# instadeepai/FrameDiPT

Hardware: AMD Instinct MI355X
Metric: residue*diffusion-steps/sec (higher is better)
Workload: dtype fp16

## Files before the change

framedipt_amd/_lib.py:

```python
from __future__ import annotations

import ctypes as C
import os

_HERE = os.path.dirname(os.path.abspath(__file__))
LIB_PATH = os.environ.get("FDIPT_LIB") or os.path.join(_HERE, "lib", "libfdipt_hip.so")

PREC_F32, PREC_BF16, PREC_F16 = 0, 1, 2
KF_ET3, KF_GENERIC_PAIR, KF_GENERIC_ATTN, KF_UNFUSED_NODE, KF_UNFOLDED, KF_NO_SPLIT, KF_NO_MERGE, KF_ROWS32, KF_PASS_Z = 1, 2, 4, 8, 16, 32, 64, 128, 256
_ERR = {-1: "FDIPT_EINVAL (bad argument)", -2: "FDIPT_ELAUNCH (HIP launch error)",
        -3: "FDIPT_ESIZE (workspace too small or N beyond the compiled tiling)"}


class FdiptError(RuntimeError):
    pass


class Dims(C.Structure):
    _fields_ = [(n, C.c_int32) for n in (
        "c_s", "c_z", "c_hidden", "c_skip", "no_heads", "no_qk_points", "no_v_points", "tfmr_heads", "tfmr_layers",
        "num_blocks", "index_embed", "num_bins", "use_aatype", "precision", "kernel_flags")] + [
        (n, C.c_float) for n in ("min_bin", "max_bin", "coordinate_scaling", "r3_min_b", "r3_max_b")]


_P = C.c_void_p


class ForwardArgs(C.Structure):
    _fields_ = [("B", C.c_int32), ("N", C.c_int32), ("n_rel", C.c_int32), ("rel_off", C.c_int32)] + [
        (n, _P) for n in ("rigids_t", "res_mask", "fixed_mask", "sc_ca_t", "seq_idx", "idx_emb", "aatype", "gt_psi", "t",
                          "t_emb", "t_emb_eps", "so3_sigma", "bb_tables", "psi", "rot_score", "trans_score", "rigids",
                          "atom37", "atom14", "trace_node", "trace_edge", "trace_inner")] + [
# ... 110 lines not shown
```

framedipt_amd/csrc/ipa_proj2.hip:

```cpp
#include <type_traits>

#include "common.hpp"
#include "kernels.hpp"

#define P2_K 256
#define P2_KS (P2_K / 16)
#define P2_WBLK (4 * P2_KS * 1024)
#define P2_XROW (P2_K * 2)
#define P2_LDS (2 * P2_WBLK)

typedef fd_h p2_hx2 __attribute__((ext_vector_type(2)));
typedef float p2_f32x2 __attribute__((ext_vector_type(2)));
typedef unsigned p2_u32x2 __attribute__((ext_vector_type(2)));
typedef unsigned p2_u32x4 __attribute__((ext_vector_type(4)));
__device__ __forceinline__ int p2_perm16(int pos) { return 4 * (pos >> 3) + (pos & 3) + 8 * ((pos & 7) >> 2); }
__device__ __forceinline__ void p2_dma16(const void* gsrc, unsigned lds_dst) {
  const unsigned m0v = __builtin_amdgcn_readfirstlane(lds_dst);
  asm volatile("s_mov_b32 m0, %0\n\ts_nop 0\n\tglobal_load_lds_dwordx4 %1, off" : : "s"(m0v), "v"(gsrc) : "memory", "m0");
}
typedef const __attribute__((address_space(3))) u16x8* p2_lds_u16x8;
typedef const __attribute__((address_space(3))) f32x4* p2_lds_f32x4;
typedef const __attribute__((address_space(3))) float* p2_lds_f32;
__device__ __forceinline__ hx8 p2_frag(unsigned off) { return __builtin_bit_cast(hx8, *(p2_lds_u16x8)(unsigned long)off); }

#define P2S_HALF 32768
#define P2S_STAGE (2 * P2S_HALF)
#define P2S_BIAS_OFF (2 * P2S_STAGE)
template <bool QK, bool SPLIT>
__device__ __forceinline__ void ipa_proj2_body(const ProjArgs& a, int n_cblk, int walker, int n_walkers, char* smem) {
  const unsigned lds0 = (unsigned)(unsigned long)(__attribute__((address_space(3))) char*)smem;
  const int tid = threadIdx.x, lane = tid & 63, wave = tid >> 6, li = lane & 31, hi = lane >> 5;
  constexpr int RB = SPLIT ? 256 : 128;
  constexpr int TM = SPLIT ? 1 : 2;
  constexpr int NTH = SPLIT ? 512 : FD_THREADS;
  const int wr = SPLIT ? wave : wave >> 1;
  int wc = SPLIT ? 0 : (wave & 1);
  const bool mrg = a.merged != 0;
  const int M = a.B * a.N, HC = a.H * a.C, NOUT = (mrg ? HC : 3 * HC) + a.PT, ntl = a.Np >> 5;
  const int m0 = blockIdx.x * RB;
  const char* wimg = (const char*)a.W_img;
  const char* wimg_lo = (const char*)a.W_img_lo;
  const int nq = HC / 128, per_head = (2 * a.C) / 128, n_class = mrg ? (QK ? nq : n_cblk - nq) : (QK ? 2 * nq : n_cblk - 2 * nq);
  auto cblk_of = [&](int k) {
    if (mrg) return QK ? k : nq + k;
    if (QK) return k < nq ? k : nq + ((k - nq) / (per_head / 2)) * per_head + (k - nq) % (per_head / 2);
    const int nv = nq;
    return k < nv ? nq + (k / (per_head / 2)) * per_head + per_head / 2 + k % (per_head / 2) : 3 * nq + (k - nv);
  };
  int kb = walker;
  auto request = [&](int c, int buf) {
// ... 60 lines not shown
    }
    __syncthreads();
  } else {
    char* xs = smem + P2_WBLK;
#pragma unroll
    for (int it = 0; it < 32; ++it) {
      const int idx = tid + it * FD_THREADS, r = idx >> 6, c4 = idx & 63;
      const int gr = m0 + r < M ? m0 + r : M - 1;
      const f32x4 x = *(const f32x4*)(a.A + (long)gr * a.lda + 4 * c4);
      const p2_u32x2 h = {fd_cvt_pk(x[0], x[1]), fd_cvt_pk(x[2], x[3])};
      *(p2_u32x2*)(xs + r * P2_XROW + (((c4 >> 1) ^ (r & 15)) << 4) + 8 * (c4 & 1)) = h;
    }
    __syncthreads();
#pragma unroll
    for (int i = 0; i < 2; ++i)
#pragma unroll
      for (int s = 0; s < P2_KS; ++s) {
        const int r = (wr * 2 + i) * 32 + li;
        Af[i][s] = p2_frag(lds0 + P2_WBLK + r * P2_XROW + (((2 * s + hi) ^ (r & 15)) << 4));
      }
    __builtin_amdgcn_s_waitcnt(0xC07F);
  }
  FD_STAMP(1);
  int qk_row[TM];
  int v_row[TM][4];
  int p_row[TM][4];
#pragma unroll
  for (int i = 0; i < TM; ++i) {
    const int m = m0 + (wr * TM + i) * 32 + li;
    const int b = m < M ? m / a.N : 0, r = m - b * a.N;
    qk_row[i] = m < M ? ((b * a.H * ntl + (r >> 5)) * (a.C >> 4) * 64 + (r & 31)) * 8 : -1;
#pragma unroll
    for (int g = 0; g < 4; ++g) {
      const int mg = m0 + (wr * TM + i) * 32 + 8 * g + 4 * hi;
      const int bb = mg < M ? mg / a.N : 0, key = mg - bb * a.N, pp = (key & ~15) + p2_perm16(key & 15);
      v_row[i][g] = mg + 3 < M ? (bb * a.H * (a.C >> 5) * (2 * ntl) + (pp >> 4)) * 512 + ((pp >> 3) & 1) * 256 + (pp & 7) : -1;
      p_row[i][g] = mg + 3 < M ? mg * a.PT : -1;
    }
  }
  auto epi_unit = [&](const f32x16 (&acc)[TM][2], const auto& BQ, const int (&cpart)[2], int kind, int i, int j, int g) {
    if constexpr (QK) {
      if ((g & 1) || qk_row[i] < 0) return;
      const f32x4 b0 = BQ.q(j, g), b1 = BQ.q(j, g + 1);
      const float sc = kind == 0 ? a.qscale : 1.f;
      const p2_u32x4 o = {fd_cvt_pk((acc[i][j][4 * g] + b0[0]) * sc, (acc[i][j][4 * g + 1] + b0[1]) * sc),
                          fd_cvt_pk((acc[i][j][4 * g + 2] + b0[2]) * sc, (acc[i][j][4 * g + 3] + b0[3]) * sc),
// ... 93 lines not shown
          acc[0][j] = fd_mfma32(l, Af[0][s], acc[0][j]);
          acc[0][j] = fd_mfma32(h, Al[0][s], acc[0][j]);
          acc[0][j] = fd_mfma32(h, Af[0][s], acc[0][j]);
        } else {
          acc[0][j] = fd_mfma32(Af[0][s], l, acc[0][j]);
          acc[0][j] = fd_mfma32(Al[0][s], h, acc[0][j]);
          acc[0][j] = fd_mfma32(Af[0][s], h, acc[0][j]);
        }
        if (has_prev && (s & 3) == 1) epi_unit(acc, bq, ep.cp, ep.kind, 0, j ^ 1, s >> 2);
        __builtin_amdgcn_sched_barrier(0);
      }
    };
    for (int hs = 0; hs < n_hs; ++hs) {
      quarter(hs, std::integral_constant<int, 0>{});
      FD_STAMP(2 + 2 * hs);
      quarter(hs, std::integral_constant<int, 1>{});
      FD_STAMP(3 + 2 * hs);
    }
    if (n_hs > 0) {
      const BiasLds bq = {cur.nb, hi, li};
#pragma unroll
      for (int g = 0; g < 4; ++g) epi_unit(acc, bq, cur.cp, cur.kind, 0, 1, g);
    }
    FD_STAMP(15);
    return;
  }
  if constexpr (!SPLIT) {
  struct BiasReg {
    f32x4 v[2][4];
    __device__ __forceinline__ f32x4 q(int j, int g) const { return v[j][g]; }
    __device__ __forceinline__ float s(int j) const { return v[j][0][0]; }
  };
  auto load_bias = [&](BiasReg& bq, int n0) {
#pragma unroll
    for (int j = 0; j < 2; ++j)
#pragma unroll
      for (int g = 0; g < 4; ++g) {
        if constexpr (QK) bq.v[j][g] = *(const f32x4*)(a.bias + n0 + (wc * 2 + j) * 32 + 16 * (g >> 1) + 8 * hi + 4 * (g & 1));
        else if (g == 0) {
          const int n = n0 + (wc * 2 + j) * 32 + li;
          bq.v[j][0][0] = n < NOUT ? a.bias[n] : 0.f;
        }
      }
  };
  auto step = [&](f32x16 (&accN)[2][2], BiasReg& bqN, int (&cpN)[2], int& kindN, const f32x16 (&accP)[2][2], const BiasReg& bqP,
                  const int (&cpP)[2], int kindP, int k, bool has_prev, int bufc) {
// ... 137 lines not shown
        const int slot = 8 * half + e, pos = 8 * ((slot >> 2) & 1) + 4 * (slot >> 3) + (slot & 3);
        const int key = 16 * s16 + pos;
        xv[e] = key < N ? node[((long)b * N + key) * ld + cc] : 0.f;
      }
      p2_u32x4 oh, ol;
#pragma unroll
      for (int q = 0; q < 4; ++q) {
        oh[q] = fd_cvt_pk(xv[2 * q], xv[2 * q + 1]);
        ol[q] = fd_cvt_pk(xv[2 * q] - h2f(f2h(xv[2 * q])), xv[2 * q + 1] - h2f(f2h(xv[2 * q + 1])));
      }
      *(p2_u32x4*)(Vt + v * 8) = oh;
      if (Vt_lo) *(p2_u32x4*)(Vt_lo + v * 8) = ol;
    }
  }
}
int fd_node_images(int B, int N, int Np, const float* node, int ld, half_t* Kb, half_t* Vt, half_t* Vt_lo, hipStream_t st) {
  if ((Np & 31) || Np < N || (ld & 3) || !Kb || !Vt) return FDIPT_EINVAL;
  const long units = (long)B * Np * 32 + (long)B * 8 * (Np / 16) * 64;
  hipLaunchKernelGGL(node_images_kernel, dim3((unsigned)((units + 255) / 256)), dim3(256), 0, st, B, N, Np, node, ld, Kb, Vt, Vt_lo);
  FD_CHECK_LAUNCH();
  return FDIPT_OK;
}

int fd_ipa_proj2_supported(const ProjArgs& a) {
  const int HC = a.H * a.C;
  return a.K == P2_K && a.W_img && (a.N & 3) == 0 && (a.C % 128) == 0 && (HC % 128) == 0 && (a.lda & 3) == 0 && (a.Np & 31) == 0 && (a.PT & 3) == 0;
}
int fd_ipa_proj2(const ProjArgs& a, hipStream_t st) {
  if (!fd_ipa_proj2_supported(a)) return FDIPT_EINVAL;
  const bool split = a.W_img_lo != nullptr;
  const int M = a.B * a.N, NOUT = (a.merged ? 1 : 3) * a.H * a.C + a.PT;
  const int n_cblk = cdiv(NOUT, 128), n_rblk = cdiv(M, split ? 256 : 128);
  const int lds = split ? P2S_BIAS_OFF + n_cblk * 128 * 4 : P2_LDS;
  if (lds > 160 * 1024 || (split && n_cblk * 128 > 8192)) return FDIPT_ESIZE;
  if (hipFuncSetAttribute(split ? (const void*)ipa_proj2_kernel<true> : (const void*)ipa_proj2_kernel<false>,
                          hipFuncAttributeMaxDynamicSharedMemorySize, lds) != hipSuccess)
    return FDIPT_ELAUNCH;
  int ncg = 256 / n_rblk;
  if (ncg < 2) ncg = 2;
  const int n_qk = (a.merged ? 1 : 2) * (a.H * a.C / 128), n_other = n_cblk - n_qk;
  int wq = (ncg * n_qk * 6 + (n_qk * 6 + n_other * 7) / 2) / (n_qk * 6 + n_other * 7);
  if (wq < 1) wq = 1;
  if (wq > ncg - 1) wq = ncg - 1;
  if (wq > n_qk) wq = n_qk;
  int wo = ncg - wq;
  if (wo > n_other) wo = n_other;
  if (split) hipLaunchKernelGGL(ipa_proj2_kernel<true>, dim3(n_rblk, wq + wo), dim3(512), lds, st, a, n_cblk, wq);
  else hipLaunchKernelGGL(ipa_proj2_kernel<false>, dim3(n_rblk, wq + wo), dim3(FD_THREADS), lds, st, a, n_cblk, wq);
  FD_CHECK_LAUNCH();
  return FDIPT_OK;
}
```

framedipt_amd/csrc/kernels.hpp:

```cpp
#pragma once
#include <hip/hip_runtime.h>
#include <stdint.h>

typedef unsigned short half_t;

struct EdgeTransArgs {
  int B, N;
  const void* z_in;
  void* z_out;
  const float* e;
  const void *w1, *w2, *wf;
  const float *b1, *b2, *bf, *gamma, *beta;
  const float* res_mask;
  float* trace;
  unsigned long long* clock = nullptr;
};

struct EdgeEmbedArgs {
  int B, N, n_rel, rel_off, num_bins;
  const float* pi;
  const float* pj;
  const float* rtab;
  const float* dtab;
  const float* edges;
// ... 113 lines not shown
size_t fd_et4_a_image_bytes(int B, int N);
size_t fd_et4_b_image_bytes(int B, int N);
int fd_et4_row_images(const float* rows, int B, int N, void* a_img, void* b_img, hipStream_t st);
int fd_edge_transition4(const ET2Args& a, hipStream_t st);
int fd_edge_transition4_supported(int N);
int fd_ee2_build_images(const float* w2, const float* w3, void* img, hipStream_t st);
size_t fd_ee2_image_bytes();
int fd_edge_embed2(const EdgeEmbedArgs& a, const void* img, hipStream_t st);

struct ProjArgs {
  int B, N, H, C, K, PT, Np;
  const float* A;
  int lda;
  const void* W;
  const void* W_img;
  const void* W_img_lo = nullptr;
  const float* bias;
  float qscale;
  half_t *Qb, *Kb, *Vt;
  half_t* Vt_lo = nullptr;
  float* pts;
  int zero_pads;
  int merged = 0;
};
int fd_node_images(int B, int N, int Np, const float* node, int ld, half_t* Kb, half_t* Vt, half_t* Vt_lo, hipStream_t st);
int fd_ipa_proj2_permute_image_q(void* img, int H, int C, int K, hipStream_t st);
int fd_ipa_proj(const ProjArgs& a, hipStream_t st);
int fd_ipa_proj_zero_pads(const ProjArgs& a, void* extra, size_t extra_bytes, hipStream_t st);
int fd_ipa_proj2_supported(const ProjArgs& a);
int fd_ipa_proj2_permute_image(void* img, int H, int C, int K, hipStream_t st);
int fd_ipa_proj2(const ProjArgs& a, hipStream_t st);

struct Attn3Args {
  int B, N, H, Np;
  const half_t *Qb, *Kb, *Vt;
  const half_t* Vt_lo = nullptr;
  int kv_per_sample = 0;
  const float* bias;
  const float* res_mask;
  const float *qp, *kp, *vp;
  const half_t* vpt;
  const half_t* kpf = nullptr;
  const float* gamma;
  const float *rot, *trans;
  float* probs;
  half_t* out_h16;
  half_t* probs_h16;
  float* out;
  long out_ld;
// ... 154 lines not shown
```

framedipt_amd/csrc/model.hip:

```cpp
#include <math.h>
#include <string.h>

#include <vector>

#include "common.hpp"
#include "kernels.hpp"

struct Switches {
  bool generic_pair = false;
  bool et3 = false;
  bool generic_attn = false;
  bool no_rowblock = false;
  bool no_chain = false;
  bool no_splitk = false;
  bool no_tail16 = false;
  bool no_et_bias = false, no_ee_bias = false;
  bool feats_unfused = false, torf_unfused = false, init_unfused = false, skip_per_block = false, post_unfused = false,
       et4_rows_unfused = false, no_pz = false;
  bool no_split = false;
  bool no_merge = false;
};
template <class IV> static bool tail16_shapes(const FdiptDims* d, const IV& iv) { return iv.d_t == 320 && d->c_s == 256; }
static Switches switches_of(const FdiptDims* d) {
  Switches s;
  const unsigned f = (unsigned)d->kernel_flags;
  if (f & FDIPT_KF_GENERIC_PAIR) s.generic_pair = true;
  if (f & FDIPT_KF_ET3) s.et3 = true;
  if (f & FDIPT_KF_GENERIC_ATTN) s.generic_attn = true;
  if (f & FDIPT_KF_UNFUSED_NODE) s.no_rowblock = s.no_chain = s.no_splitk = true;
  if (f & FDIPT_KF_NO_SPLIT) s.no_split = true;
  if (f & FDIPT_KF_NO_MERGE) s.no_merge = true;
  if (f & FDIPT_KF_ROWS32) s.no_tail16 = true;
  if (f & FDIPT_KF_PASS_Z) s.no_pz = true;
  if (f & FDIPT_KF_UNFOLDED)
    s.no_et_bias = s.no_ee_bias = s.feats_unfused = s.torf_unfused = s.init_unfused = s.skip_per_block = s.post_unfused =
        s.et4_rows_unfused = true;
  return s;
}

struct LinW { long w, b; int out, in; };
struct LNW { long g, b; int d; };
#define FD_MAX_BLOCKS 8
#define FD_MAX_TL 4
struct TfLayer { LinW inp, outp, l1, l2; LNW n1, n2; };
struct BlockW {
  long head_w;
  LinW q, kv, qp, kvp, lb, dz, out, rbf;
  LNW ipa_ln;
  LinW skip;
  TfLayer tf[FD_MAX_TL];
  LinW post, t1, t2, t3;
  LNW tln;
  LinW bb;
  LinW et_init, et1, et2, etf;
  LNW et_ln;
};
// ... 47 lines not shown
    k.t1 = lin(cs, cs); k.t2 = lin(cs, cs); k.t3 = lin(cs, cs); k.tln = ln(cs);
    k.bb = lin(6, cs);
    if (b < d->num_blocks - 1) {
      k.et_init = lin(iv.cb, cs); k.et1 = lin(iv.hid, iv.hid); k.et2 = lin(iv.hid, iv.hid); k.etf = lin(cz, iv.hid);
      k.et_ln = ln(cz);
    }
  }
  iv.tor1 = lin(cs, cs); iv.tor2 = lin(cs, cs); iv.tor3 = lin(cs, cs); iv.torf = lin(2, cs);
  iv.offsets.push_back(off);
}

static inline size_t al256(size_t x) { return (x + 255) & ~(size_t)255; }
static inline int rup8(int x) { return (x + 7) & ~7; }

struct DSplit {
  size_t inp[FD_MAX_TL], outp[FD_MAX_TL], l1[FD_MAX_TL], l2[FD_MAX_TL], post, t1, t2, t3, et_init, r4w;
  size_t o16[FD_MAX_TL][2], f16[FD_MAX_TL][2], g16[FD_MAX_TL][2], p16[2];
  size_t tr16[3][2];
  size_t ei16[2], r416[2];
};
struct DChain {
  size_t skip, inp[FD_MAX_TL], outp[FD_MAX_TL], l1[FD_MAX_TL], l2[FD_MAX_TL], l2n[FD_MAX_TL], post, t1, t2, t3, t2n, t3n, et_init, a1, af, a1af, b1f, r4w, r4b;
};
struct DBlock { size_t wq_m, wproj2_img, wproj2_img_lo, bproj2, wout_m, bout_m, wout_img, wout_img_lo, wproj, wproj_img, wproj_img_lo, bproj, gamma, wb, bb, wb_img3, wb_img4, et3, et4, wdz_t, wdz_img, wdz_img_lo, wdz_imgp, wdz_imgp_lo; DChain ch; DSplit lo; };
struct DLayout {
  size_t h16_base;
  size_t ne0_pad;
  size_t w1i, w1j, w1r, dtab, edges, b1;
  size_t ee2;
  size_t ch_ne0, ch_ne2, ch_ne4, ch_tor1, ch_tor2;
  size_t ch_ne2n, ch_ne4n, ch_tor2n;
  size_t lo_ne0, lo_ne2, lo_ne4, lo_tor1, lo_tor2;
  size_t skip16[2];
  size_t ne16[3][2], tor16[2][2];
  size_t skip_w32;
  size_t skip_w, skip_b;
  DBlock blk[FD_MAX_BLOCKS];
  size_t total;
  int kn_pad, d1_pad, esz;
};

static bool use_regpair(const FdiptDims* d) {
  return d->precision == FDIPT_PREC_HALF && d->c_z == 128 && d->c_s == 256 && !switches_of(d).generic_pair;
}

static bool use_chain(const FdiptDims* d) {
  return d->precision == FDIPT_PREC_HALF && d->c_s == 256 && d->c_skip == 64 && d->c_z == 128 && !switches_of(d).no_chain;
// ... 8 lines not shown
  if (d->precision == FDIPT_PREC_HALF) o = al256(o + (size_t)iv.offsets.back() * 2);
  L.ne0_pad = o; o = al256(o + (size_t)d->c_s * L.kn_pad * L.esz);
  L.w1i = o; o = al256(o + (size_t)d->c_z * L.d1_pad * 4);
  L.w1j = o; o = al256(o + (size_t)d->c_z * L.d1_pad * 4);
  L.w1r = o; o = al256(o + (size_t)d->c_z * d->index_embed * 4);
  L.dtab = o; o = al256(o + (size_t)(d->num_bins + 1) * d->c_z * 4);
  L.edges = o; o = al256(o + (size_t)d->num_bins * 4);
  L.b1 = o; o = al256(o + (size_t)d->c_z * 4);
  L.ee2 = o;
  if (use_regpair(d)) o = al256(o + fd_ee2_image_bytes());
  for (int b = 0; b < d->num_blocks; ++b) {
    L.blk[b].wproj = o; o = al256(o + (size_t)iv.proj_out * d->c_s * L.esz);
    L.blk[b].wproj_img = o;
    if (L.esz == 2 && d->c_s == 256) o = al256(o + (size_t)((iv.proj_out + 127) / 128) * 65536);
    L.blk[b].wproj_img_lo = o;
    if (L.esz == 2 && d->c_s == 256) o = al256(o + (size_t)((iv.proj_out + 127) / 128) * 65536);
    L.blk[b].bproj = o; o = al256(o + (size_t)iv.proj_out * 4);
    {
      const int HCm = d->no_heads * d->c_hidden, n2 = iv.proj_out - 2 * HCm;
      L.blk[b].wq_m = o; o = al256(o + (size_t)HCm * d->c_s * 4);
      L.blk[b].wproj2_img = o; if (L.esz == 2 && d->c_s == 256) o = al256(o + (size_t)((n2 + 127) / 128) * 65536);
      L.blk[b].wproj2_img_lo = o; if (L.esz == 2 && d->c_s == 256) o = al256(o + (size_t)((n2 + 127) / 128) * 65536);
      L.blk[b].bproj2 = o; o = al256(o + (size_t)n2 * 4);
      L.blk[b].wout_m = o; o = al256(o + (size_t)d->c_s * iv.feat_dim * 4);
      L.blk[b].bout_m = o; o = al256(o + (size_t)d->c_s * 4);
      L.blk[b].wout_img = o; if (fd_outproj_split_supported(d->c_s, iv.feat_dim)) o = al256(o + fd_chain_image_bytes(d->c_s, iv.feat_dim));
      L.blk[b].wout_img_lo = o; if (fd_outproj_split_supported(d->c_s, iv.feat_dim)) o = al256(o + fd_chain_image_bytes(d->c_s, iv.feat_dim));
    }
    L.blk[b].gamma = o; o = al256(o + (size_t)d->no_heads * 4);
    L.blk[b].wb = o; o = al256(o + (size_t)d->no_heads * d->c_z * L.esz);
    L.blk[b].bb = o; o = al256(o + (size_t)d->no_heads * 4);
    L.blk[b].wb_img3 = o; o = al256(o + 4096);
    L.blk[b].wb_img4 = o; o = al256(o + 8192);
    L.blk[b].wdz_img = o; o = al256(o + 8192);
    L.blk[b].wdz_img_lo = o; o = al256(o + 8192);
    L.blk[b].wdz_imgp = o; o = al256(o + 8192);
    L.blk[b].wdz_imgp_lo = o; o = al256(o + 8192);
    L.blk[b].wdz_t = o; o = al256(o + (size_t)d->c_z * (d->c_z / 4) * 4);
    L.blk[b].et3 = o;
    if (use_regpair(d) && b < d->num_blocks - 1) o = al256(o + fd_et3_stream_bytes());
    L.blk[b].et4 = o;
    if (use_regpair(d) && b < d->num_blocks - 1) o = al256(o + fd_et4_stream_bytes());
    if (use_chain(d)) {
      DChain& c = L.blk[b].ch;
      auto img = [&](int n, int k) { size_t r = o; o = al256(o + fd_chain_image_bytes(n, k)); return r; };
      const int cs = d->c_s, dt = iv.d_t;
// ... 201 lines not shown
                         (float*)(D + db.wout_m), (float*)(D + db.bout_m));
      FD_CHECK_LAUNCH();
      if (fd_outproj_split_supported(cs, iv.feat_dim) &&
          ((rc = fd_chain_build_image((const float*)(D + db.wout_m), cs, iv.feat_dim, iv.feat_dim, 0, D + db.wout_img, st)) ||
           (rc = fd_chain_build_image_lo((const float*)(D + db.wout_m), cs, iv.feat_dim, iv.feat_dim, D + db.wout_img_lo, st))))
        return rc;
      const int HCm = H * C, n2 = iv.proj_out - 2 * HCm;
      if ((rc = copy_cols(4, 1, k.qp.out, k.qp.out, P + k.qp.b, k.qp.out, 0, 1.f, D + db.bproj2 + (size_t)HCm * 4, st)) ||
          (rc = copy_cols(4, 1, k.kvp.out, k.kvp.out, P + k.kvp.b, k.kvp.out, 0, 1.f, D + db.bproj2 + (size_t)(HCm + k.qp.out) * 4, st)))
        return rc;
      if (proj_img && C % 128 == 0 && HCm % 128 == 0 && k.qp.out % 32 == 0 && k.kvp.out % 32 == 0) {
        const size_t ib = (size_t)((n2 + 127) / 128) * 65536, tile = (size_t)(cs / 16) * 1024;
        if (hipMemsetAsync(D + db.wproj2_img, 0, ib, st) != hipSuccess || hipMemsetAsync(D + db.wproj2_img_lo, 0, ib, st) != hipSuccess) return FDIPT_ELAUNCH;
        const float* srcs[3] = {(const float*)(D + db.wq_m), P + k.qp.w, P + k.kvp.w};
        const int rows[3] = {HCm, k.qp.out, k.kvp.out};
        long r0 = 0;
        for (int p3 = 0; p3 < 3; ++p3) {
          if ((rc = fd_chain_build_image(srcs[p3], rows[p3], cs, cs, 0, D + db.wproj2_img + (size_t)(r0 / 32) * tile, st)) ||
              (rc = fd_chain_build_image_lo(srcs[p3], rows[p3], cs, cs, D + db.wproj2_img_lo + (size_t)(r0 / 32) * tile, st)))
            return rc;
          r0 += rows[p3];
        }
        if ((rc = fd_ipa_proj2_permute_image_q(D + db.wproj2_img, H, C, cs, st)) || (rc = fd_ipa_proj2_permute_image_q(D + db.wproj2_img_lo, H, C, cs, st)))
          return rc;
      }
    }
    hipLaunchKernelGGL(gamma_kernel, dim3(1), dim3(64), 0, st, H, d->no_qk_points, P + k.head_w, (float*)(D + db.gamma));
    FD_CHECK_LAUNCH();
    if ((rc = copy_cols(L.esz, H, cz, cz, P + k.lb.w, cz, 0, s3, D + db.wb, st))) return rc;
    if ((rc = copy_cols(4, 1, H, H, P + k.lb.b, H, 0, s3, D + db.bb, st))) return rc;
    if (cz == 128 && H <= 8)
      if ((rc = fd_et3_build_bias_image(P + k.lb.w, H, s3, D + db.wb_img3, st)) ||
          (rc = fd_et4_build_bias_image(P + k.lb.w, H, s3, D + db.wb_img4, st)))
        return rc;
    hipLaunchKernelGGL(transpose_kernel, dim3(16), dim3(256), 0, st, cz / 4, cz, P + k.dz.w, (float*)(D + db.wdz_t));
    FD_CHECK_LAUNCH();
    if (cz == 128 && ((rc = fd_chain_build_image(P + k.dz.w, cz / 4, cz, cz, 0, D + db.wdz_img, st)) ||
                      (rc = fd_chain_build_image_lo(P + k.dz.w, cz / 4, cz, cz, D + db.wdz_img_lo, st)) ||
                      (rc = fd_chain_build_image_ex(P + k.dz.w, cz / 4, cz, cz, 1, 0, D + db.wdz_imgp, st)) ||
                      (rc = fd_chain_build_image_ex(P + k.dz.w, cz / 4, cz, cz, 1, 1, D + db.wdz_imgp_lo, st))))
      return rc;
    if (b > 0 && cz == 128 && use_regpair(d) && (rc = fd_et4_set_dz(D + L.blk[b - 1].et4, D + db.wdz_imgp, D + db.wdz_imgp_lo, st))) return rc;
    if (use_regpair(d) && b < d->num_blocks - 1)
      if ((rc = fd_et3_build_stream(P + k.et1.w, P + k.et2.w, P + k.etf.w, D + db.et3, st)) ||
          (rc = fd_et4_build_stream(P + k.et1.w, P + k.et2.w, P + k.etf.w, D + db.et4, st)))
        return rc;
// ... 410 lines not shown
    oa.wdz = (const float*)(D + db.wdz_t); oa.wdz_img = (bf && cz == 128) ? D + db.wdz_img : nullptr; oa.wdz_img_lo = (oa.wdz_img && split) ? D + db.wdz_img_lo : nullptr; oa.bdz = P + k.dz.b;
    bool feats_h16 = false, skip_done = false, merged = false;
    const bool use_a3 = ipa.a3;
    PointsArgs pa;
    pa.B = B; pa.N = N; pa.H = H; pa.Pq = Pq; pa.Pv = Pv; pa.quat = F(w.quat); pa.trans = F(w.trans);
    pa.qp = F(w.qp); pa.kp = F(w.kp); pa.vp = F(w.vp); pa.rot = F(w.rot);
    pa.vpt = (use_a3 && Pv == 12) ? (unsigned short*)(W + w.vpt) : nullptr; pa.Np = Np;
    if (use_a3) { pa.kpf = (unsigned short*)(W + w.kpf); pa.gamma = (const float*)(D + db.gamma); pa.res_mask = res_mask; }
    const size_t vpt_bytes = (size_t)B * H * 96 * Np * 2;
    bool vpt_zero = pa.vpt && (b == 0 || op.kind != OP_ALL);
    if (use_a3) {
      ProjArgs pj;
      pj.B = B; pj.N = N; pj.H = H; pj.C = C; pj.K = cs; pj.PT = PT; pj.Np = Np; pj.A = node_cur; pj.lda = cs;
      pj.W = D + db.wproj; pj.bias = (const float*)(D + db.bproj); pj.qscale = sqrtf(1.0f / (3.0f * (float)C));
      pj.Qb = (half_t*)(W + w.qb); pj.Kb = (half_t*)(W + w.kb); pj.Vt = (half_t*)(W + w.vt); pj.pts = F(w.pts);
      pj.zero_pads = b == 0 || op.kind != OP_ALL;
      pj.W_img = cs == 256 ? D + db.wproj_img : nullptr;
      pj.W_img_lo = (pj.W_img && split) ? D + db.wproj_img_lo : nullptr;
      merged = pj.W_img_lo && split && cs == C && !sw.no_merge && op.kind == OP_ALL && fd_ipa_proj2_supported(pj);
      if (merged) {
        pj.merged = 1; pj.W_img = D + db.wproj2_img; pj.W_img_lo = D + db.wproj2_img_lo; pj.bias = (const float*)(D + db.bproj2);
        a3.kv_per_sample = 1;
        if (split) a3.Vt_lo = (const half_t*)(W + w.vt_lo);
      } else if (pj.W_img_lo && split && fd_ipa_proj2_supported(pj)) {
        pj.Vt_lo = (half_t*)(W + w.vt_lo); a3.Vt_lo = pj.Vt_lo;
      }
      if (fd_ipa_proj2_supported(pj)) {
        if (pj.zero_pads && seq_fused && !seq_img_ready && (C & 31) == 0 && (vpt_bytes & 15) == 0 && !sw.init_unfused) {
          SeqInitExtra sx = {vpt_zero ? W + w.vpt : nullptr, vpt_zero ? (long)(vpt_bytes >> 4) : 0L, (Np > N && !merged) ? (void*)pj.Kb : nullptr,
                             (void*)pj.Vt, (long)B * H, C, (void*)pj.Vt_lo};
          RC(fd_seq_images_init(B, N, d->tfmr_heads, res_mask, W + w.seqimg, sx, st));
          seq_img_ready = true;
          vpt_zero = false;
        } else if (pj.zero_pads && ((Np > N && !merged) || vpt_zero)) {
          ProjArgs pz = pj; pz.W_img = nullptr;
          if (merged) pz.Np = pz.N;
          RC(fd_ipa_proj_zero_pads(pz, vpt_zero ? W + w.vpt : nullptr, vpt_zero ? vpt_bytes : 0, st));
          vpt_zero = false;
        }
        RC(fd_ipa_proj2(pj, st));
        if (merged) {
          if (pa.vpt && Pv == 12 && (H & 1) == 0 && cs == 256) {
            pa.node = node_cur; pa.ld_node = cs; pa.nKb = pj.Kb; pa.nVt = pj.Vt; pa.nVt_lo = split ? (half_t*)(W + w.vt_lo) : nullptr;
          } else RC(fd_node_images(B, N, Np, node_cur, cs, pj.Kb, pj.Vt, split ? (half_t*)(W + w.vt_lo) : nullptr, st));
        }
      } else RC(fd_ipa_proj(pj, st));
      if (vpt_zero && hipMemsetAsync(W + w.vpt, 0, vpt_bytes, st) != hipSuccess) return FDIPT_ELAUNCH;
      pa.proj = F(w.pts); pa.ld = PT; pa.q_off = 0; pa.kv_off = 3 * H * Pq;
      RC(fd_points(pa, st));
      if (op.kind == OP_POINTS) return FD_STOP;
      if (!bias_ready)
        RC(fd_pair_bias2(B, N, H, W + w.z, D + db.wb, (const float*)(D + db.bb), F(w.bias), 1, st));
      feats_h16 = fd_opair_mfma_eligible(prec, oa) && iv.feat_dim >= 1024 && (iv.feat_dim & 7) == 0 && !sw.no_splitk &&
                   !split && op.kind == OP_ALL;
      if (feats_h16) { a3.out_h16 = (half_t*)(W + w.feats); oa.out_h16 = a3.out_h16; }
      if (ipa.probs_h16) {
        a3.probs_h16 = (half_t*)(W + w.probs); oa.probs_h16 = a3.probs_h16; oa.probs_np = Np;
      }
      RC(fd_attention3(a3, st));
    } else {
      RC(fd_linear(prec, R, iv.proj_out, cs, node_cur, cs, D + db.wproj, cs, (const float*)(D + db.bproj), nullptr, 0,
                   nullptr, 0, F(w.proj), iv.proj_out, st));
      pa.proj = F(w.proj); pa.ld = iv.proj_out; pa.q_off = 3 * H * C; pa.kv_off = 3 * H * C + 3 * H * Pq;
      RC(fd_points(pa, st));
      if (op.kind == OP_POINTS) return FD_STOP;
      AttnArgs aa;
      aa.B = B; aa.N = N; aa.H = H;
      aa.q = F(w.proj); aa.q_ld = iv.proj_out; aa.q_hs = C;
      aa.k = F(w.proj) + H * C; aa.k_ld = iv.proj_out; aa.k_hs = 2 * C;
      aa.v = F(w.proj) + H * C + C; aa.v_ld = iv.proj_out; aa.v_hs = 2 * C;
      aa.C = C; aa.Dv = C; aa.scale = sqrtf(1.0f / (3.0f * (float)C));
      aa.bias = F(w.bias); aa.res_mask = res_mask; aa.qp = F(w.qp); aa.kp = F(w.kp); aa.vp = F(w.vp); aa.Pq = Pq; aa.Pv = Pv;
// ... 362 lines not shown
```

include/fdipt.h:

```cpp
#ifndef FDIPT_H
#define FDIPT_H

#include <stddef.h>
#include <stdint.h>

#ifdef __cplusplus
extern "C" {
#endif

#define FDIPT_OK 0
#define FDIPT_EINVAL (-1)
#define FDIPT_ELAUNCH (-2)
#define FDIPT_ESIZE (-3)

#define FDIPT_PREC_F32 0
#define FDIPT_PREC_BF16 1
#define FDIPT_PREC_F16 2

#define FDIPT_KF_ET3 1
#define FDIPT_KF_GENERIC_PAIR 2
#define FDIPT_KF_GENERIC_ATTN 4
#define FDIPT_KF_UNFUSED_NODE 8
#define FDIPT_KF_UNFOLDED 16
#define FDIPT_KF_NO_SPLIT 32
#define FDIPT_KF_NO_MERGE 64
#define FDIPT_KF_ROWS32 128
#define FDIPT_KF_PASS_Z 256
#define FDIPT_KF_ALL 511

typedef void* fdipt_stream_t;

typedef struct FdiptDims {
  int32_t c_s;
  int32_t c_z;
  int32_t c_hidden;
  int32_t c_skip;
  int32_t no_heads;
  int32_t no_qk_points;
  int32_t no_v_points;
  int32_t tfmr_heads;
  int32_t tfmr_layers;
  int32_t num_blocks;
  int32_t index_embed;
  int32_t num_bins;
  int32_t use_aatype;
  int32_t precision;
  int32_t kernel_flags;
  float min_bin;
  float max_bin;
  float coordinate_scaling;
  float r3_min_b;
// ... 170 lines not shown
```

Before: 1.116 million.

## Fuse IPA point rotation and key/value image packing into merged projection kernel

Folds the separate points kernel into the split-precision IPA projection GEMM. A permuted weight image reorders the point columns so each walker block can rotate its query, key and value points by the residue frames in LDS. It then writes the packed kpf/vpt attention images, the rotation matrices and the query points directly. Node K/V images are also emitted from the projection kernel instead of a separate pass. This removes a kernel launch and a round trip of the point projections through global memory, at the cost of extra LDS, more kernel complexity, extra weight images, and a new kernel flag to fall back to the old path.

Result: faster. 1.147 million, median of 6 (+2.7%).

```diff
diff --git a/framedipt_amd/_lib.py b/framedipt_amd/_lib.py
--- a/framedipt_amd/_lib.py
+++ b/framedipt_amd/_lib.py
@@ -8,6 +8,7 @@
 
 PREC_F32, PREC_BF16, PREC_F16 = 0, 1, 2
 KF_ET3, KF_GENERIC_PAIR, KF_GENERIC_ATTN, KF_UNFUSED_NODE, KF_UNFOLDED, KF_NO_SPLIT, KF_NO_MERGE, KF_ROWS32, KF_PASS_Z = 1, 2, 4, 8, 16, 32, 64, 128, 256
+KF_POINTS_LAUNCH = 512
 _ERR = {-1: "FDIPT_EINVAL (bad argument)", -2: "FDIPT_ELAUNCH (HIP launch error)",
         -3: "FDIPT_ESIZE (workspace too small or N beyond the compiled tiling)"}
 
diff --git a/framedipt_amd/csrc/ipa_proj2.hip b/framedipt_amd/csrc/ipa_proj2.hip
--- a/framedipt_amd/csrc/ipa_proj2.hip
+++ b/framedipt_amd/csrc/ipa_proj2.hip
@@ -26,6 +26,253 @@
 #define P2S_HALF 32768
 #define P2S_STAGE (2 * P2S_HALF)
 #define P2S_BIAS_OFF (2 * P2S_STAGE)
+__host__ __device__ __forceinline__ int p2p_src_col(int n) {
+  const int c = n >> 7, col = n & 127;
+  if (c < 4) {
+    if (col < 72) { const int vh = col / 36, r = col % 36; return 192 + (r % 3) * 160 + (2 * c + vh) * 20 + 8 + r / 3; }
+    if (col < 120) { const int r = col - 72, kh = r / 24, q = r % 24; return 192 + (q % 3) * 160 + (2 * c + kh) * 20 + q / 3; }
+    return -1;
+  }
+  if (c > 5 || col >= 96) return -1;
+  const int hq = col / 24, r = col % 24;
+  return (r % 3) * 64 + (4 * (c - 4) + hq) * 8 + r / 3;
+}
+#define P2P_COLS 768
+typedef __attribute__((address_space(3))) f32x4* p2_lds_f32x4w;
+typedef __attribute__((address_space(3))) u16x8* p2_lds_u16x8w;
+typedef const __attribute__((address_space(3))) unsigned* p2_lds_u32;
+
+__device__ __forceinline__ void p2_kpf_units(const ProjArgs& a, const float (&kv)[24], bool lv, int b, int h, int key, int ntl) {
+#pragma unroll
+  for (int un = 0; un < 8; ++un) {
+    const int f = un >> 1, hf = un & 1;
+    unsigned short o[8];
+    if (f == 3 && hf == 1) {
+      float kn = 0.f;
+      if (lv)
+#pragma unroll
+        for (int c = 0; c < 24; ++c) kn = fmaf(kv[c], kv[c], kn);
+      const float m = lv ? a.res_mask[(long)b * a.N + key] : 0.f;
+      const float t0 = fmaxf(-0.5f * a.gamma[h] * kn, -65000.f);
+      const unsigned short p0 = f2f16(t0);
+      const float t1 = t0 - f162f(p0);
+      const unsigned short p1 = f2f16(t1);
+      const unsigned short p2 = f2f16(t1 - f162f(p1));
+      o[0] = f2f16(2.f * m); o[1] = f2f16(m); o[2] = f2f16(lv ? 0.f : -60000.f); o[3] = p0; o[4] = p1; o[5] = p2; o[6] = o[7] = 0;
+    } else {
+      const int c0 = f < 2 ? 8 * hf : 16;
+      const bool lo = f == 1 || (f == 2 && hf == 1);
+#pragma unroll
+      for (int e = 0; e < 8; ++e) {
+        const float x = lv ? kv[c0 + e] : 0.f;
+        const unsigned short xh = f2f16(x);
+        o[e] = lo ? f2f16(x - f162f(xh)) : xh;
+      }
+    }
+    const p2_u32x4 val = {o[0] | ((unsigned)o[1] << 16), o[2] | ((unsigned)o[3] << 16), o[4] | ((unsigned)o[5] << 16), o[6] | ((unsigned)o[7] << 16)};
+    *(p2_u32x4*)(a.kpf + ((((((long)b * a.H + h) * ntl + (key >> 5)) * FD_KPF_FRAGS + f) * 64 + hf * 32 + (key & 31)) << 3)) = val;
+  }
+}
+
+template <class RQ>
+__device__ __forceinline__ void p2_points_walk(const ProjArgs& a, const hx8 (&Af)[P2_KS], const hx8 (&Al)[P2_KS], int n_class, int nq, int walker,
+                                               int n_walkers, unsigned lds0, unsigned fr, RQ& request_half) {
+  const int tid = threadIdx.x, lane = tid & 63, wave = tid >> 6, li = lane & 31, hi = lane >> 5;
+  const int M = a.B * a.N, m0 = blockIdx.x * 256, H = a.H, ntl = a.Np >> 5, ks = a.Np >> 4;
+  auto tile_at = [&](int col, int rg) { return lds0 + (unsigned)(col * 1024 + ((rg ^ (col & 63)) << 4)); };
+  auto rotate = [&](int row, float px, float py, float pz, float* g3) {
+    float R[12];
+#pragma unroll
+    for (int i = 0; i < 12; ++i) R[i] = *(p2_lds_f32)(unsigned long)(fr + 4 * (i * 256 + row));
+    g3[0] = R[0] * px + R[1] * py + R[2] * pz + R[9];
+    g3[1] = R[3] * px + R[4] * py + R[5] * pz + R[10];
+    g3[2] = R[6] * px + R[7] * py + R[8] * pz + R[11];
+  };
+  for (int k = walker; k < n_class; k += n_walkers) {
+    const int c = nq + k;
+    const bool frames = k == walker && tid < 256;
+    f32x4 fq = {0.f, 0.f, 0.f, 0.f};
+    float ft[3] = {0.f, 0.f, 0.f};
+    if (frames) {
+      const int gr = m0 + tid < M ? m0 + tid : M - 1;
+      fq = *(const f32x4*)(a.quat + (long)gr * 4);
+#pragma unroll
+      for (int d = 0; d < 3; ++d) ft[d] = a.trans[(long)gr * 3 + d];
+    }
+    __syncthreads();
+    request_half(c, 0, 0);
+    request_half(c, 1, 1);
+#pragma unroll 1
+    for (int half = 0; half < 2; ++half) {
+      if (half == 0) __builtin_amdgcn_s_waitcnt(0x0F78);
+      else __builtin_amdgcn_s_waitcnt(0x0F70);
+      if (half == 0 && frames) {
+        const float w = fq[0], x = fq[1], y = fq[2], z = fq[3];
+        float R[9];
+        R[0] = w * w + x * x - y * y - z * z; R[1] = 2 * x * y - 2 * w * z; R[2] = 2 * x * z + 2 * w * y;
+        R[3] = 2 * x * y + 2 * w * z; R[4] = w * w - x * x + y * y - z * z; R[5] = 2 * y * z - 2 * w * x;
+        R[6] = 2 * x * z - 2 * w * y; R[7] = 2 * y * z + 2 * w * x; R[8] = w * w - x * x - y * y + z * z;
+#pragma unroll
+        for (int i = 0; i < 12; ++i) *(__attribute__((address_space(3))) float*)(unsigned long)(fr + 4 * (i * 256 + tid)) = i < 9 ? R[i] : ft[i - 9];
+        if (walker == 0 && m0 + tid < M)
+#pragma unroll
+          for (int i = 0; i < 9; ++i) a.rot[(long)(m0 + tid) * 9 + i] = R[i];
+      }
+      __syncthreads();
+      f32x16 acc[2];
+#pragma unroll
+      for (int j = 0; j < 2; ++j) {
+#pragma unroll
+        for (int r = 0; r < 16; ++r) acc[j][r] = 0.f;
+        const unsigned wbh = lds0 + half * P2S_STAGE + j * (P2_KS * 1024) + lane * 16, wbl = wbh + P2S_HALF;
+        constexpr int DEPTH = 3;
+        hx8 wh[DEPTH], wl[DEPTH];
+#pragma unroll
+        for (int s = 0; s < DEPTH - 1; ++s) { wh[s] = p2_frag(wbh + s * 1024); wl[s] = p2_frag(wbl + s * 1024); }
+        __builtin_amdgcn_sched_barrier(0);
+#pragma unroll
+        for (int s = 0; s < P2_KS; ++s) {
+          if (s + DEPTH - 1 < P2_KS) {
+            wh[(s + DEPTH - 1) % DEPTH] = p2_frag(wbh + (s + DEPTH - 1) * 1024);
+            wl[(s + DEPTH - 1) % DEPTH] = p2_frag(wbl + (s + DEPTH - 1) * 1024);
+          }
+          const hx8 h = wh[s % DEPTH], l = wl[s % DEPTH];
+          acc[j] = fd_mfma32(Af[s], l, acc[j]);
+          acc[j] = fd_mfma32(Al[s], h, acc[j]);
+          acc[j] = fd_mfma32(Af[s], h, acc[j]);
+          __builtin_amdgcn_sched_barrier(0);
+        }
+      }
+      float bv[2];
+#pragma unroll
+      for (int j = 0; j < 2; ++j) bv[j] = *(p2_lds_f32)(unsigned long)(lds0 + P2S_BIAS_OFF + 4 * (c * 128 + 64 * half + 32 * j + li));
+      __syncthreads();
+#pragma unroll
+      for (int j = 0; j < 2; ++j)
+#pragma unroll
+        for (int g = 0; g < 4; ++g) {
+          const f32x4 v = {acc[j][4 * g] + bv[j], acc[j][4 * g + 1] + bv[j], acc[j][4 * g + 2] + bv[j], acc[j][4 * g + 3] + bv[j]};
+          *(p2_lds_f32x4w)(unsigned long)tile_at(64 * half + 32 * j + li, 8 * wave + 2 * g + hi) = v;
+        }
+    }
+    __syncthreads();
+    auto tv = [&](int row, int col) { return *(p2_lds_f32)(unsigned long)(tile_at(col, row >> 2) + 4 * (row & 3)); };
+    int tid = threadIdx.x;
+    asm volatile("" : "+v"(tid));
+    if (k < 4) {
+      {
+        const int row = tid & 255, kh = tid >> 8, m = m0 + row;
+        if (m < M) {
+          const int b = m / a.N, key = m - b * a.N;
+          float kv[24];
+#pragma unroll
+          for (int e = 0; e < 8; ++e) {
+            const int col = 72 + 24 * kh + 3 * e;
+            rotate(row, tv(row, col), tv(row, col + 1), tv(row, col + 2), kv + 3 * e);
+          }
+          p2_kpf_units(a, kv, true, b, 2 * k + kh, key, ntl);
+        }
+        const int npad = a.Np - a.N;
+        if (npad > 0)
+          for (int bs = m0 / a.N; bs < a.B && bs * a.N < m0 + 256; ++bs) {
+            const int end = bs * a.N + a.N - 1;
+            if (end < m0 || end >= m0 + 256) continue;
+            float z[24];
+#pragma unroll
+            for (int q = 0; q < 24; ++q) z[q] = 0.f;
+#pragma unroll 1
+            for (int u = tid; u < 2 * npad; u += 512) p2_kpf_units(a, z, false, bs, 2 * k + (u & 1), a.N + (u >> 1), ntl);
+          }
+      }
+#pragma unroll 1
+      for (int t = tid; t < 64 * 24; t += 512) {
+        const int k4 = t & 63, rest = t >> 6, vh = rest / 12, e = rest - 12 * vh, mg = m0 + 4 * k4;
+        if (mg >= M) continue;
+        const int b = mg / a.N, key = mg - b * a.N, pp = (key & ~15) + p2_perm16(key & 15), h = 2 * k + vh;
+        f32x4 pc[3];
+#pragma unroll
+        for (int d = 0; d < 3; ++d) pc[d] = *(p2_lds_f32x4)(unsigned long)tile_at(36 * vh + 3 * e + d, k4);
+        unsigned short vhs[3][4], vls[3][4];
+#pragma unroll
+        for (int q = 0; q < 4; ++q) {
+          float g3[3];
+          rotate(4 * k4 + q, pc[0][q], pc[1][q], pc[2][q], g3);
+#pragma unroll
+          for (int d = 0; d < 3; ++d) {
+            const unsigned short vh16 = f2h(g3[d]);
+            vhs[d][q] = vh16;
+            vls[d][q] = f2h(g3[d] - h2f(vh16));
+          }
+        }
+#pragma unroll
+        for (int d = 0; d < 3; ++d) {
+          const int rw = 3 * e + d, rl = 36 + rw;
+          const long bh3 = ((long)b * H + h) * 3;
+          const long oh = ((((bh3 + (rw >> 5)) * ks + (pp >> 4)) * 64 + ((pp >> 3) & 1) * 32 + (rw & 31)) << 3) + (pp & 7);
+          const long ol = ((((bh3 + (rl >> 5)) * ks + (pp >> 4)) * 64 + ((pp >> 3) & 1) * 32 + (rl & 31)) << 3) + (pp & 7);
+          *(p2_u32x2*)(a.vpt + oh) = p2_u32x2{vhs[d][0] | ((unsigned)vhs[d][1] << 16), vhs[d][2] | ((unsigned)vhs[d][3] << 16)};
+          *(p2_u32x2*)(a.vpt + ol) = p2_u32x2{vls[d][0] | ((unsigned)vls[d][1] << 16), vls[d][2] | ((unsigned)vls[d][3] << 16)};
+        }
+      }
+    } else {
+#pragma unroll 1
+      for (int t = tid; t < 1024; t += 512) {
+        const int row = t & 255, hq = t >> 8, m = m0 + row;
+        if (m >= M) continue;
+        float g[24];
+#pragma unroll
+        for (int e = 0; e < 8; ++e) {
+          const int col = 24 * hq + 3 * e;
+          rotate(row, tv(row, col), tv(row, col + 1), tv(row, col + 2), g + 3 * e);
+        }
+        float* dst = a.qp + ((long)m * H * 8 + (4 * (k - 4) + hq) * 8) * 3;
+#pragma unroll
+        for (int v = 0; v < 6; ++v) *(f32x4*)(dst + 4 * v) = f32x4{g[4 * v], g[4 * v + 1], g[4 * v + 2], g[4 * v + 3]};
+      }
+    }
+  }
+}
+
+__device__ __forceinline__ void p2_node_rows(const ProjArgs& a, const hx8 (&Af)[P2_KS], const hx8 (&Al)[P2_KS], int walker, int n_walkers,
+                                             unsigned lds0) {
+  const int tid = threadIdx.x, lane = tid & 63, wave = tid >> 6, li = lane & 31, hi = lane >> 5;
+  const int M = a.B * a.N, mw = blockIdx.x * 256 + wave * 32, ntl = a.Np >> 5;
+  for (int p = walker; p < 3; p += n_walkers) {
+    if (p == 0) {
+      const int m = mw + li;
+      if (m < M) {
+        const int b = m / a.N, r = m - b * a.N;
+        half_t* dst = a.Kb + ((((long)b * ntl + (r >> 5)) * 16) * 64 + hi * 32 + (r & 31)) * 8;
+#pragma unroll
+        for (int s = 0; s < P2_KS; ++s) *(hx8*)(dst + s * 64 * 8) = Af[s];
+      }
+      continue;
+    }
+    __syncthreads();
+    const unsigned xl = lds0 + wave * (32 * P2_XROW);
+#pragma unroll
+    for (int s = 0; s < P2_KS; ++s)
+      *(p2_lds_u16x8w)(unsigned long)(xl + li * P2_XROW + (((2 * s + hi) ^ (li & 15)) << 4)) = __builtin_bit_cast(u16x8, p == 1 ? Af[s] : Al[s]);
+    __builtin_amdgcn_s_waitcnt(0xC07F);
+    half_t* img = p == 1 ? a.Vt : a.Vt_lo;
+#pragma unroll 4
+    for (int t = 0; t < 16; ++t) {
+      const int task = t * 64 + lane, cc = 2 * (task & 127), k4 = task >> 7, mg = mw + 4 * k4;
+      unsigned w[4];
+#pragma unroll
+      for (int q = 0; q < 4; ++q) {
+        const int rr = 4 * k4 + q;
+        w[q] = *(p2_lds_u32)(unsigned long)(xl + rr * P2_XROW + (((cc >> 3) ^ (rr & 15)) << 4) + (cc & 7) * 2);
+      }
+      if (mg >= M) continue;
+      const int b = mg / a.N, key = mg - b * a.N, pp = (key & ~15) + p2_perm16(key & 15);
+      const long u0 = ((((long)b * 8 + (cc >> 5)) * (2 * ntl) + (pp >> 4)) * 64 + ((pp >> 3) & 1) * 32 + (cc & 31)) * 8 + (pp & 7);
+      *(p2_u32x2*)(img + u0) = p2_u32x2{(w[0] & 0xffffu) | (w[1] << 16), (w[2] & 0xffffu) | (w[3] << 16)};
+      *(p2_u32x2*)(img + u0 + 8) = p2_u32x2{(w[0] >> 16) | (w[1] & 0xffff0000u), (w[2] >> 16) | (w[3] & 0xffff0000u)};
+    }
+  }
+}
+
 template <bool QK, bool SPLIT>
 __device__ __forceinline__ void ipa_proj2_body(const ProjArgs& a, int n_cblk, int walker, int n_walkers, char* smem) {
   const unsigned lds0 = (unsigned)(unsigned long)(__attribute__((address_space(3))) char*)smem;
@@ -132,6 +379,12 @@
     __builtin_amdgcn_s_waitcnt(0xC07F);
   }
   FD_STAMP(1);
+  if constexpr (SPLIT && !QK) {
+    if (a.pts_img) {
+      p2_points_walk(a, Af[0], Al[0], n_class, nq, kb, n_walkers, lds0, lds0 + P2S_BIAS_OFF + n_cblk * 512, request_half);
+      return;
+    }
+  }
   int qk_row[TM];
   int v_row[TM][4];
   int p_row[TM][4];
@@ -271,6 +524,8 @@
 #pragma unroll
       for (int g = 0; g < 4; ++g) epi_unit(acc, bq, cur.cp, cur.kind, 0, 1, g);
     }
+    if constexpr (QK)
+      if (a.pts_img) p2_node_rows(a, Af[0], Al[0], walker, n_walkers, lds0);
     FD_STAMP(15);
     return;
   }
@@ -454,6 +709,36 @@
   return FDIPT_OK;
 }
 
+__global__ void p2_points_image_kernel(const u16x8* __restrict__ src, const float* __restrict__ sbias, u16x8* __restrict__ dst,
+                                       float* __restrict__ dbias, int HC, int ks) {
+  const long n_units = (long)(HC + P2P_COLS) / 32 * ks * 64;
+  for (long u = blockIdx.x * (long)blockDim.x + threadIdx.x; u < n_units; u += (long)gridDim.x * blockDim.x) {
+    const int lane = (int)(u & 63), s = (int)((u >> 6) % ks), t = (int)(u / (64L * ks));
+    int n = 32 * t + (lane & 31);
+    if (n >= HC) {
+      const int o = p2p_src_col(n - HC);
+      n = o < 0 ? -1 : HC + o;
+    }
+    dst[u] = n < 0 ? u16x8{0, 0, 0, 0, 0, 0, 0, 0} : src[((long)(n >> 5) * ks + s) * 64 + (n & 31) + 32 * (lane >> 5)];
+    if (s == 0 && lane < 32) {
+      const int j = 32 * t + lane;
+      dbias[j] = n < 0 ? 0.f : sbias[n];
+    }
+  }
+}
+int fd_ipa_proj2_points_cols(int H, int C) { return H * C + P2P_COLS; }
+int fd_ipa_proj2_points_image(const void* src_img, const float* src_bias, void* img, float* bias, int H, int C, int K, hipStream_t st) {
+  if (H != 8 || C != 256 || (K & 15)) return FDIPT_EINVAL;
+  const long units = (long)fd_ipa_proj2_points_cols(H, C) / 32 * (K / 16) * 64;
+  hipLaunchKernelGGL(p2_points_image_kernel, dim3((unsigned)((units + 255) / 256)), dim3(256), 0, st, (const u16x8*)src_img, src_bias,
+                     (u16x8*)img, bias, H * C, K / 16);
+  FD_CHECK_LAUNCH();
+  return FDIPT_OK;
+}
+int fd_ipa_proj2_points_supported(const ProjArgs& a, int Pq, int Pv) {
+  return a.merged && a.W_img && a.W_img_lo && a.H == 8 && a.C == 256 && a.K == 256 && Pq == 8 && Pv == 12 &&
+         a.PT == 3 * a.H * (2 * Pq + Pv) && (a.N & 3) == 0 && (a.Np & 31) == 0 && a.Np >= a.N && (a.lda & 3) == 0;
+}
 int fd_ipa_proj2_supported(const ProjArgs& a) {
   const int HC = a.H * a.C;
   return a.K == P2_K && a.W_img && (a.N & 3) == 0 && (a.C % 128) == 0 && (HC % 128) == 0 && (a.lda & 3) == 0 && (a.Np & 31) == 0 && (a.PT & 3) == 0;
@@ -463,7 +748,10 @@
   const bool split = a.W_img_lo != nullptr;
   const int M = a.B * a.N, NOUT = (a.merged ? 1 : 3) * a.H * a.C + a.PT;
   const int n_cblk = cdiv(NOUT, 128), n_rblk = cdiv(M, split ? 256 : 128);
-  const int lds = split ? P2S_BIAS_OFF + n_cblk * 128 * 4 : P2_LDS;
+  if (a.pts_img && (!split || !a.merged || a.PT != P2P_COLS || a.H != 8 || a.C != 256 || !a.quat || !a.trans || !a.rot || !a.qp || !a.kpf ||
+                    !a.vpt || !a.gamma || !a.res_mask || !a.Kb || !a.Vt || !a.Vt_lo))
+    return FDIPT_EINVAL;
+  const int lds = split ? P2S_BIAS_OFF + n_cblk * 128 * 4 + (a.pts_img ? 12 * 256 * 4 : 0) : P2_LDS;
   if (lds > 160 * 1024 || (split && n_cblk * 128 > 8192)) return FDIPT_ESIZE;
   if (hipFuncSetAttribute(split ? (const void*)ipa_proj2_kernel<true> : (const void*)ipa_proj2_kernel<false>,
                           hipFuncAttributeMaxDynamicSharedMemorySize, lds) != hipSuccess)
diff --git a/framedipt_amd/csrc/kernels.hpp b/framedipt_amd/csrc/kernels.hpp
--- a/framedipt_amd/csrc/kernels.hpp
+++ b/framedipt_amd/csrc/kernels.hpp
@@ -159,9 +159,19 @@
   float* pts;
   int zero_pads;
   int merged = 0;
+  int pts_img = 0;
+  const float* quat = nullptr;
+  const float* trans = nullptr;
+  const float* gamma = nullptr;
+  const float* res_mask = nullptr;
+  float *rot = nullptr, *qp = nullptr;
+  unsigned short *kpf = nullptr, *vpt = nullptr;
 };
 int fd_node_images(int B, int N, int Np, const float* node, int ld, half_t* Kb, half_t* Vt, half_t* Vt_lo, hipStream_t st);
 int fd_ipa_proj2_permute_image_q(void* img, int H, int C, int K, hipStream_t st);
+int fd_ipa_proj2_points_supported(const ProjArgs& a, int Pq, int Pv);
+int fd_ipa_proj2_points_cols(int H, int C);
+int fd_ipa_proj2_points_image(const void* src_img, const float* src_bias, void* img, float* bias, int H, int C, int K, hipStream_t st);
 int fd_ipa_proj(const ProjArgs& a, hipStream_t st);
 int fd_ipa_proj_zero_pads(const ProjArgs& a, void* extra, size_t extra_bytes, hipStream_t st);
 int fd_ipa_proj2_supported(const ProjArgs& a);
diff --git a/framedipt_amd/csrc/model.hip b/framedipt_amd/csrc/model.hip
--- a/framedipt_amd/csrc/model.hip
+++ b/framedipt_amd/csrc/model.hip
@@ -19,6 +19,7 @@
        et4_rows_unfused = false, no_pz = false;
   bool no_split = false;
   bool no_merge = false;
+  bool points_launch = false;
 };
 template <class IV> static bool tail16_shapes(const FdiptDims* d, const IV& iv) { return iv.d_t == 320 && d->c_s == 256; }
 static Switches switches_of(const FdiptDims* d) {
@@ -32,6 +33,7 @@
   if (f & FDIPT_KF_NO_MERGE) s.no_merge = true;
   if (f & FDIPT_KF_ROWS32) s.no_tail16 = true;
   if (f & FDIPT_KF_PASS_Z) s.no_pz = true;
+  if (f & FDIPT_KF_POINTS_LAUNCH) s.points_launch = true;
   if (f & FDIPT_KF_UNFOLDED)
     s.no_et_bias = s.no_ee_bias = s.feats_unfused = s.torf_unfused = s.init_unfused = s.skip_per_block = s.post_unfused =
         s.et4_rows_unfused = true;
@@ -125,7 +127,7 @@
 struct DChain {
   size_t skip, inp[FD_MAX_TL], outp[FD_MAX_TL], l1[FD_MAX_TL], l2[FD_MAX_TL], l2n[FD_MAX_TL], post, t1, t2, t3, t2n, t3n, et_init, a1, af, a1af, b1f, r4w, r4b;
 };
-struct DBlock { size_t wq_m, wproj2_img, wproj2_img_lo, bproj2, wout_m, bout_m, wout_img, wout_img_lo, wproj, wproj_img, wproj_img_lo, bproj, gamma, wb, bb, wb_img3, wb_img4, et3, et4, wdz_t, wdz_img, wdz_img_lo, wdz_imgp, wdz_imgp_lo; DChain ch; DSplit lo; };
+struct DBlock { size_t wq_m, wproj2_img, wproj2_img_lo, bproj2, wproj2p_img, wproj2p_img_lo, bproj2p, wout_m, bout_m, wout_img, wout_img_lo, wproj, wproj_img, wproj_img_lo, bproj, gamma, wb, bb, wb_img3, wb_img4, et3, et4, wdz_t, wdz_img, wdz_img_lo, wdz_imgp, wdz_imgp_lo; DChain ch; DSplit lo; };
 struct DLayout {
   size_t h16_base;
   size_t ne0_pad;
@@ -180,6 +182,11 @@
       L.blk[b].wproj2_img = o; if (L.esz == 2 && d->c_s == 256) o = al256(o + (size_t)((n2 + 127) / 128) * 65536);
       L.blk[b].wproj2_img_lo = o; if (L.esz == 2 && d->c_s == 256) o = al256(o + (size_t)((n2 + 127) / 128) * 65536);
       L.blk[b].bproj2 = o; o = al256(o + (size_t)n2 * 4);
+      const bool pimg = L.esz == 2 && d->c_s == 256 && d->c_hidden == 256 && d->no_heads == 8;
+      const size_t pcols = pimg ? (size_t)fd_ipa_proj2_points_cols(d->no_heads, d->c_hidden) : 0;
+      L.blk[b].wproj2p_img = o; o = al256(o + pcols / 128 * 65536);
+      L.blk[b].wproj2p_img_lo = o; o = al256(o + pcols / 128 * 65536);
+      L.blk[b].bproj2p = o; o = al256(o + pcols * 4);
       L.blk[b].wout_m = o; o = al256(o + (size_t)d->c_s * iv.feat_dim * 4);
       L.blk[b].bout_m = o; o = al256(o + (size_t)d->c_s * 4);
       L.blk[b].wout_img = o; if (fd_outproj_split_supported(d->c_s, iv.feat_dim)) o = al256(o + fd_chain_image_bytes(d->c_s, iv.feat_dim));
@@ -427,6 +434,10 @@
           r0 += rows[p3];
         }
         if ((rc = fd_ipa_proj2_permute_image_q(D + db.wproj2_img, H, C, cs, st)) || (rc = fd_ipa_proj2_permute_image_q(D + db.wproj2_img_lo, H, C, cs, st)))
+          return rc;
+        if (H == 8 && C == 256 && cs == 256 && d->no_qk_points == 8 && d->no_v_points == 12 &&
+            ((rc = fd_ipa_proj2_points_image(D + db.wproj2_img, (const float*)(D + db.bproj2), D + db.wproj2p_img, (float*)(D + db.bproj2p), H, C, cs, st)) ||
+             (rc = fd_ipa_proj2_points_image(D + db.wproj2_img_lo, (const float*)(D + db.bproj2), D + db.wproj2p_img_lo, (float*)(D + db.bproj2p), H, C, cs, st))))
           return rc;
       }
     }
@@ -883,24 +894,32 @@
         pj.merged = 1; pj.W_img = D + db.wproj2_img; pj.W_img_lo = D + db.wproj2_img_lo; pj.bias = (const float*)(D + db.bproj2);
         a3.kv_per_sample = 1;
         if (split) a3.Vt_lo = (const half_t*)(W + w.vt_lo);
-      } else if (pj.W_img_lo && split && fd_ipa_proj2_supported(pj)) {
+      }
+      const bool proj_pts = merged && !sw.points_launch && pa.vpt && pa.kpf && fd_ipa_proj2_points_supported(pj, Pq, Pv);
+      if (proj_pts) {
+        pj.pts_img = 1; pj.W_img = D + db.wproj2p_img; pj.W_img_lo = D + db.wproj2p_img_lo; pj.bias = (const float*)(D + db.bproj2p);
+        pj.PT = fd_ipa_proj2_points_cols(H, C) - H * C; pj.Vt_lo = (half_t*)(W + w.vt_lo);
+        pj.quat = pa.quat; pj.trans = pa.trans; pj.gamma = pa.gamma; pj.res_mask = pa.res_mask; pj.rot = pa.rot; pj.qp = pa.qp;
+        pj.kpf = pa.kpf; pj.vpt = pa.vpt;
+      }
+      if (!merged && pj.W_img_lo && split && fd_ipa_proj2_supported(pj)) {
         pj.Vt_lo = (half_t*)(W + w.vt_lo); a3.Vt_lo = pj.Vt_lo;
       }
       if (fd_ipa_proj2_supported(pj)) {
         if (pj.zero_pads && seq_fused && !seq_img_ready && (C & 31) == 0 && (vpt_bytes & 15) == 0 && !sw.init_unfused) {
-          SeqInitExtra sx = {vpt_zero ? W + w.vpt : nullptr, vpt_zero ? (long)(vpt_bytes >> 4) : 0L, (Np > N && !merged) ? (void*)pj.Kb : nullptr,
+          SeqInitExtra sx = {vpt_zero ? W + w.vpt : nullptr, vpt_zero ? (long)(vpt_bytes >> 4) : 0L, (Np > N && (!merged || proj_pts)) ? (void*)pj.Kb : nullptr,
                              (void*)pj.Vt, (long)B * H, C, (void*)pj.Vt_lo};
           RC(fd_seq_images_init(B, N, d->tfmr_heads, res_mask, W + w.seqimg, sx, st));
           seq_img_ready = true;
           vpt_zero = false;
-        } else if (pj.zero_pads && ((Np > N && !merged) || vpt_zero)) {
+        } else if (pj.zero_pads && ((Np > N && (!merged || proj_pts)) || vpt_zero)) {
           ProjArgs pz = pj; pz.W_img = nullptr;
-          if (merged) pz.Np = pz.N;
+          if (merged && !proj_pts) pz.Np = pz.N;
           RC(fd_ipa_proj_zero_pads(pz, vpt_zero ? W + w.vpt : nullptr, vpt_zero ? vpt_bytes : 0, st));
           vpt_zero = false;
         }
         RC(fd_ipa_proj2(pj, st));
-        if (merged) {
+        if (merged && !proj_pts) {
           if (pa.vpt && Pv == 12 && (H & 1) == 0 && cs == 256) {
             pa.node = node_cur; pa.ld_node = cs; pa.nKb = pj.Kb; pa.nVt = pj.Vt; pa.nVt_lo = split ? (half_t*)(W + w.vt_lo) : nullptr;
           } else RC(fd_node_images(B, N, Np, node_cur, cs, pj.Kb, pj.Vt, split ? (half_t*)(W + w.vt_lo) : nullptr, st));
@@ -908,7 +927,7 @@
       } else RC(fd_ipa_proj(pj, st));
       if (vpt_zero && hipMemsetAsync(W + w.vpt, 0, vpt_bytes, st) != hipSuccess) return FDIPT_ELAUNCH;
       pa.proj = F(w.pts); pa.ld = PT; pa.q_off = 0; pa.kv_off = 3 * H * Pq;
-      RC(fd_points(pa, st));
+      if (!proj_pts) RC(fd_points(pa, st));
       if (op.kind == OP_POINTS) return FD_STOP;
       if (!bias_ready)
         RC(fd_pair_bias2(B, N, H, W + w.z, D + db.wb, (const float*)(D + db.bb), F(w.bias), 1, st));
diff --git a/include/fdipt.h b/include/fdipt.h
--- a/include/fdipt.h
+++ b/include/fdipt.h
@@ -26,7 +26,8 @@
 #define FDIPT_KF_NO_MERGE 64
 #define FDIPT_KF_ROWS32 128
 #define FDIPT_KF_PASS_Z 256
-#define FDIPT_KF_ALL 511
+#define FDIPT_KF_POINTS_LAUNCH 512
+#define FDIPT_KF_ALL 1023
 
 typedef void* fdipt_stream_t;
 
```
